# FitSNAP/FitSNAP

Measured on AMD Instinct MI355X. Metric: training rows/sec through A^T A + solve, 1000000 x 128 fp64 in total over the GPUs (strong scaling), higher is better.
Workload: dtype f64

## Files before the change

fitsnap_amd/build.py:

```python
from __future__ import annotations

import hashlib
import os
import shutil
import subprocess
import sys

HERE = os.path.dirname(os.path.abspath(__file__))
CSRC = os.path.join(HERE, "csrc")
LIBDIR = os.path.join(HERE, "_lib")
LIBNAME = "libfsnap_hip.so"
SOURCES = ["fsnap_syrk_quad.hip:0", "fsnap_syrk_quad.hip:1", "fsnap_syrk_quad.hip:2", "fsnap_syrk.hip", "fsnap_syrk_short.hip", "fsnap_rows.hip", "fsnap_chol.hip", "fsnap_trsm.hip", "fsnap_fused.hip", "fsnap_merr.hip", "fsnap_cand.hip", "fsnap_uq.hip", "fsnap_loco.hip", "fsnap_path.hip", "fsnap_joint.hip", "fsnap_select.hip", "fsnap_mcmc.hip", "fsnap_capi.cpp", "fsnap_comm.cpp", "fsnap_p2p.cpp",
           "fsnap_rowspace.cpp", "fsnap_rowspace_host.cpp", "fsnap_solve.cpp"]
HEADERS = ["fsnap_kernels.h", "fsnap_device_common.h", "fsnap_rowvar_body.h", "fsnap_ctx.h", "fsnap_rowspace_host.h", "fsnap_condest.h", "fsnap_p2p.h", os.path.join("..", "..", "include", "fsnap_hip.h")]
ARCH = "gfx950"


def lib_path() -> str:
    return os.path.join(LIBDIR, LIBNAME)


def _hipcc() -> str:
    exe = shutil.which("hipcc") or "/opt/rocm/bin/hipcc"
    if not os.path.exists(exe):
        raise RuntimeError("hipcc not found: libfsnap_hip.so cannot be built")
    return exe


def _source_digest() -> str:
    h = hashlib.sha256()
    for name in sorted({s.split(":")[0] for s in SOURCES}) + HEADERS:
        with open(os.path.join(CSRC, name), "rb") as f:
            h.update(f.read())
    return h.hexdigest()


def build_library(force: bool = False, verbose: bool = False) -> str:
    os.makedirs(LIBDIR, exist_ok=True)
    out = lib_path()
    stamp = out + ".sha256"
    digest = _source_digest()
    if not force and os.path.exists(out) and os.path.exists(stamp):
        with open(stamp) as f:
            if f.read().strip() == digest:
                return out
    hipcc = _hipcc()
    objs = []
    common = [f"--offload-arch={ARCH}", "-O3", "-std=c++17", "-fPIC", "-I", os.path.join(HERE, "..", "include")]
    procs = []
    objdir = os.path.join(LIBDIR, "obj")
    os.makedirs(objdir, exist_ok=True)
    hh = hashlib.sha256()
    for name in HEADERS:
        with open(os.path.join(CSRC, name), "rb") as f:
            hh.update(f.read())
    for entry in SOURCES:
        src, _, part = entry.partition(":")
        obj = os.path.join(objdir, os.path.splitext(src)[0] + (f"_{part}" if part else "") + ".o")
        cmd = [hipcc, *common]
        if part:
            cmd += [f"-DFSNAP_QUAD_PART={part}"]
        if src in ("fsnap_capi.cpp", "fsnap_comm.cpp", "fsnap_p2p.cpp", "fsnap_rowspace.cpp"):
            cmd += ["-x", "hip"]
        if src in ("fsnap_solve.cpp", "fsnap_rowspace_host.cpp"):
            cmd = [hipcc, "-x", "c++", "-O3", "-std=c++17", "-fPIC", "-mavx2", "-mfma",
                   "-I", os.path.join(HERE, "..", "include")]
        cmd += ["-c", os.path.join(CSRC, src), "-o", obj]
# ... 37 lines not shown
```

fitsnap_amd/csrc/fsnap_capi.cpp:

```cpp
#include <hip/hip_runtime.h>

#include <algorithm>
#include <cmath>
#include <atomic>
#include <chrono>
#include <cstdarg>
#include <cstdio>
#include <cstdlib>
#include <cstring>
#include <limits>
#include <new>
#include <queue>
#include <string>
#include <thread>
#include <vector>

#include "../../include/fsnap_hip.h"
#include "fsnap_kernels.h"

extern "C" int fsnap_solve_diag_tagged(int kind, double param, int64_t K, const double* G, const double* c, const double* diag,
                                       double* beta, int* rank, double* rcond_est, int upper, const void* owner,
                                       unsigned long long generation);
extern "C" int fsnap_solve_diag_upper(int kind, double param, int64_t K, const double* G, const double* c, const double* diag,
                                      double* beta, int* rank, double* rcond_est);
// ... 455 lines not shown
    return FSNAP_OK;
}

int launch_normal_eq_tiled(fsnap_ctx* ctx, double* d_packed, bool accumulate) {
    int rc;
    TiledGeometry g;
    if ((rc = plan_tiled(ctx, &g))) return rc;
    int npk = 0;
    if ((rc = ensure_wpack(ctx, &npk))) return rc;
    if (!ctx->part.ensure((size_t)g.nsplit * g.npairs * 4096 * sizeof(double)) ||
        !ctx->cpart.ensure((size_t)g.nsplit * g.NSB * 4 * 64 * sizeof(double)))
        return ctx->fail(FSNAP_E_NOMEM, "hipMalloc(partials) failed");
    fsnap::TiledArgs a;
    a.A = ctx->dA;
    a.lda = ctx->lda;
    a.wpack = ctx->wpack_override ? ctx->wpack_override : (const double*)ctx->wpack.p;
    a.m = ctx->m;
    a.K = (int)ctx->K;
    a.NSB = g.NSB;
    a.npairs = g.npairs;
    a.nsplit = g.nsplit;
    a.chunks_per_split = g.cps;
    a.nontemporal = false;
    a.part = (double*)ctx->part.p;
    a.cpart = (double*)ctx->cpart.p;
    a.spart = (const double*)ctx->wpack_spart.p;
    a.ns = npk;
    const int64_t cpart_key = ((int64_t)g.nsplit << 32) | (int64_t)g.NSB;
    if (ctx->cpart_key != cpart_key || ctx->cpart_ptr != ctx->cpart.p) {
        FSNAP_HIP(hipMemsetAsync(a.cpart, 0, (size_t)g.nsplit * g.NSB * 4 * 64 * sizeof(double), ctx->stream), "hipMemsetAsync");
        ctx->cpart_key = cpart_key;
        ctx->cpart_ptr = ctx->cpart.p;
    }
    hipEvent_t* evs;
    if ((rc = fit_events(ctx, &evs))) return rc;
    if (evs) FSNAP_HIP(hipEventRecord(evs[0], ctx->stream), "hipEventRecord");
    FSNAP_HIP(fsnap::launch_syrk_tiled(a, ctx->stream), "launch fsnap_syrk_tiled");
    if (evs) FSNAP_HIP(hipEventRecord(evs[1], ctx->stream), "hipEventRecord");
    FSNAP_HIP(fsnap::launch_reduce_tiled(a, d_packed, accumulate, ctx->stream), "launch fsnap_reduce_tiled");
    if (evs) FSNAP_HIP(hipEventRecord(evs[2], ctx->stream), "hipEventRecord");
    if (evs) ctx->t_syrk = true;
    return FSNAP_OK;
}

int launch_normal_eq(fsnap_ctx* ctx, double* d_packed, bool want_mirror = false, bool accumulate = false) {
    int rc;
    ctx->mirror_of = nullptr;
    ctx->chol_factor_of = nullptr;
    if ((rc = check_rows(ctx)) || (rc = check_weights(ctx))) return rc;
    if (use_tiled(ctx)) return launch_normal_eq_tiled(ctx, d_packed, accumulate);
    Geometry g;
    if ((rc = plan_geometry(ctx, &g))) return rc;
    const unsigned char* mask = ctx->dmask;
    if (!mask) {
        if ((rc = ensure_ones(ctx))) return rc;
        mask = (const unsigned char*)ctx->ones.p;
    }
    const int NT = g.NB * (g.NB + 1) / 2;
    const int cs_per_block = g.shortk ? 1 : 4 * g.cluster;
    if (!ctx->part.ensure((size_t)g.nblocks * NT * 256 * sizeof(double)) ||
        !ctx->cpart.ensure((size_t)g.nblocks * cs_per_block * g.NB * 16 * sizeof(double)) ||
        !ctx->spart.ensure((size_t)g.nblocks * cs_per_block * 4 * sizeof(double)))
        return ctx->fail(FSNAP_E_NOMEM, "hipMalloc(partials) failed");
    fsnap::SyrkArgs a;
    a.A = ctx->dA;
    a.lda = ctx->lda;
    a.b = ctx->db;
    a.w = ctx->dw;
    a.mask = mask;
    a.m = ctx->m;
    a.K = (int)ctx->K;
    a.nblocks = g.nblocks;
    a.split = g.split;
    a.chunks_per_wave = g.cpw;
    a.nontemporal = true;
    a.part = (double*)ctx->part.p;
    a.cpart = (double*)ctx->cpart.p;
    a.spart = (double*)ctx->spart.p;
    int ns = -1;
    const double* spart_src = a.spart;
    if (g.fused_pack) {
        a.fused_pack = true;
    } else {
        int npk = 0;
        if ((rc = ensure_wpack(ctx, &npk))) return rc;
        a.wpack = ctx->wpack_override ? ctx->wpack_override : (const double*)ctx->wpack.p;
        spart_src = (const double*)ctx->wpack_spart.p;
        ns = npk;
    }
    hipEvent_t* evs;
    if ((rc = fit_events(ctx, &evs))) return rc;
    if (evs) FSNAP_HIP(hipEventRecord(evs[0], ctx->stream), "hipEventRecord");
    if (g.quad && g.cluster > 1) {
        const size_t need = (size_t)g.nblocks * 4 * sizeof(int);
        if (ctx->quad_flow.bytes < need) {
            if (!ctx->quad_flow.ensure(need)) return ctx->fail(FSNAP_E_NOMEM, "hipMalloc(flow words) failed");
            FSNAP_HIP(hipMemsetAsync(ctx->quad_flow.p, 0, ctx->quad_flow.bytes, ctx->stream), "hipMemset(flow words)");
            ctx->quad_flow_tag = 0;
        }
        ctx->quad_flow_tag += 1u << 20;
        a.flow_words = (int*)ctx->quad_flow.p;
        const int flow = 2 | ((g.cluster == 2 ? 0 : 2) << 2);
        a.flow_tag = (int)(ctx->quad_flow_tag | (unsigned)flow);
    }
    if (g.shortk) FSNAP_HIP(fsnap::launch_syrk_short(a, ctx->stream), "launch fsnap_syrk_short");
    else if (g.quad) FSNAP_HIP(fsnap::launch_syrk_quad(a, ctx->stream), "launch fsnap_syrk_quad");
    else if (g.acc) FSNAP_HIP(fsnap::launch_syrk_acc(a, ctx->stream), "launch fsnap_syrk_acc");
// ... 2253 lines not shown
```

fitsnap_amd/csrc/fsnap_syrk.hip:

```cpp

#include <utility>

#include "fsnap_device_common.h"
#include "fsnap_kernels.h"

namespace {

__host__ __device__ constexpr int tri_index(int p, int q, int NB) {
    return p * NB - (p * (p - 1)) / 2 + (q - p);
}

__host__ __device__ inline int col_of(int bq, int e, int NB) {
    if ((NB & 1) && bq == NB - 1) return 16 * bq + e;
    return 32 * (bq >> 1) + 2 * e + (bq & 1);
}

__device__ __forceinline__ __amdgpu_buffer_rsrc_t make_rsrc(const void* p, unsigned bytes) {
    return __builtin_amdgcn_make_buffer_rsrc(const_cast<void*>(p), 0, (int)bytes, 0x00020000);
}

__device__ __forceinline__ double xlane_sum_rows(double x) {
    x += __shfl_xor(x, 16, 64);
    x += __shfl_xor(x, 32, 64);
    return x;
}

}

#ifdef FSNAP_TRACE
__device__ unsigned long long fsnap_trace_buf[4096 * 8];
__device__ unsigned long long fsnap_trace_wave[4096 * 16 * 4];
#define FSNAP_TRACE_CLK(v) const unsigned long long v = __builtin_readcyclecounter()
#endif

namespace {

template <int T, int NV>
__device__ __forceinline__ void acc_mfma(double a, double b, d4 (&vt)[NV]) {
    if constexpr (T < 32) {
        asm volatile("v_mfma_f64_16x16x4_f64 a[%2:%3], %0, %1, a[%2:%3]" : : "v"(a), "v"(b), "n"(8 * T), "n"(8 * T + 7));
    } else {
        asm volatile("v_mfma_f64_16x16x4_f64 %0, %1, %2, %0" : "+v"(vt[T - 32]) : "v"(a), "v"(b));
    }
}

template <int R>
__device__ __forceinline__ void acc_zero_reg() {
    asm volatile("v_accvgpr_write_b32 a[%0], 0" : : "n"(R));
}
template <int... R>
__device__ __forceinline__ void acc_zero_all(std::integer_sequence<int, R...>) {
    (acc_zero_reg<R>(), ...);
}

template <int T, int NV>
__device__ __forceinline__ d4 acc_read(const d4 (&vt)[NV]) {
    if constexpr (T >= 32) {
// ... 29 lines not shown

template <int NB>
struct RawM {
    u4 pr[NB / 2 > 0 ? NB / 2 : 1];
    u2 tail;
    u4 wp;
};

constexpr unsigned FSNAP_OOB_VOFF = 0xFFFFF000u;

struct WaveBufsP {
    __amdgpu_buffer_rsrc_t A, wp;
    unsigned voffA;
    unsigned voffT;
    unsigned voffP;
    unsigned chunk_bytes;
};

__device__ __forceinline__ u4 load_pack(const WaveBufsP& wb, unsigned cl) {
    return __builtin_amdgcn_raw_buffer_load_b128(wb.wp, wb.voffP, cl * 64u, 0);
}
__device__ __forceinline__ bool pack_keep(const u4& wp) {
    return ((wp[0] | (wp[1] & 0x7FFFFFFFu)) != 0u);
}

template <int NB, bool NT>
__device__ __forceinline__ void issue_rows(RawM<NB>& r, const WaveBufsP& wb, unsigned cl) {
    const unsigned soff = cl * wb.chunk_bytes;
    constexpr int AUX = NT ? 2 : 0;
    const bool keep = pack_keep(r.wp);
    const unsigned va = keep ? wb.voffA : FSNAP_OOB_VOFF;
#pragma unroll
    for (int j = 0; j < NB / 2; ++j) r.pr[j] = __builtin_amdgcn_raw_buffer_load_b128(wb.A, va + 256u * j, soff, AUX);
    if (NB & 1) {
        const unsigned vtl = keep ? wb.voffT : FSNAP_OOB_VOFF;
        r.tail = __builtin_amdgcn_raw_buffer_load_b64(wb.A, vtl, soff, AUX);
    }
}

template <int NB, bool NT>
__device__ __forceinline__ void issue_rows_w(RawM<NB>& r, const u4& wp, const WaveBufsP& wb, unsigned cl) {
    const unsigned soff = cl * wb.chunk_bytes;
    constexpr int AUX = NT ? 2 : 0;
    const bool keep = pack_keep(wp);
    const unsigned va = keep ? wb.voffA : FSNAP_OOB_VOFF;
#pragma unroll
    for (int j = 0; j < NB / 2; ++j) r.pr[j] = __builtin_amdgcn_raw_buffer_load_b128(wb.A, va + 256u * j, soff, AUX);
    if (NB & 1) {
        const unsigned vtl = keep ? wb.voffT : FSNAP_OOB_VOFF;
        r.tail = __builtin_amdgcn_raw_buffer_load_b64(wb.A, vtl, soff, AUX);
    }
}

template <class F, int... I>
__device__ __forceinline__ void wave_p_for_impl(F&& f, std::integer_sequence<int, I...>) {
    (f(std::integral_constant<int, I>{}), ...);
}
template <int N, class F>
__device__ __forceinline__ void wave_p_for(F&& f) {
    wave_p_for_impl(f, std::make_integer_sequence<int, N>{});
}

template <int NB, bool NT, int P>
__device__ __forceinline__ void issue_piece(RawM<NB>& r, const WaveBufsP& wb, unsigned cl, unsigned va, unsigned vtl) {
    constexpr int AUX = NT ? 2 : 0;
    constexpr int NPR = NB / 2;
    const unsigned soff = cl * wb.chunk_bytes;
    if (P < NPR) r.pr[P] = __builtin_amdgcn_raw_buffer_load_b128(wb.A, va + 256u * P, soff, AUX);
    if ((NB & 1) && P == NPR) r.tail = __builtin_amdgcn_raw_buffer_load_b64(wb.A, vtl, soff, AUX);
    static_assert(NPR + (NB & 1) <= NB, "one load piece per MFMA slot");
}

template <int NB, bool FULLK>
__device__ __forceinline__ double weighted_block(const RawM<NB>& r, int j, double wv, int K, int e) {
    if ((NB & 1) && j == NB - 1) {
        const double x = wv * __builtin_bit_cast(double, r.tail);
        if (FULLK) return x;
        return (16 * (NB - 1) + e < K) ? x : 0.0;
    }
    const double x = wv * __builtin_bit_cast(d2, r.pr[j >> 1])[j & 1];
    constexpr int last_pair = (NB & 1) ? -1 : NB / 2 - 1;
    if (FULLK || (j >> 1) != last_pair) return x;
    return (32 * (j >> 1) + 2 * e + (j & 1) < K) ? x : 0.0;
}

template <bool PACK>
__device__ __forceinline__ u4 load_pack_x(const WaveBufsP& wb, const double* lpk, unsigned cl) {
    if constexpr (PACK) return __builtin_bit_cast(u4, *reinterpret_cast<const d2*>(lpk + (size_t)cl * 8));
    else return load_pack(wb, cl);
}

__device__ __forceinline__ void pack_rows_to_lds(const double* __restrict__ b, const double* __restrict__ w,
                                                 const unsigned char* __restrict__ mask, int64_t row0, int64_t nrow,
                                                 unsigned wave_rows, unsigned region_rows, double* lpw, int lane, double* sout) {
    constexpr int PB = 16;
    const __amdgpu_buffer_rsrc_t rb = make_rsrc(b + row0, (unsigned)(nrow * 8));
    const __amdgpu_buffer_rsrc_t rw_ = make_rsrc(w + row0, (unsigned)(nrow * 8));
    const __amdgpu_buffer_rsrc_t rm = make_rsrc(mask + row0, (unsigned)nrow);
    double bb = 0.0, sb = 0.0, cnt = 0.0;
    for (unsigned r0 = 0; r0 < wave_rows; r0 += 64u * PB) {
        u2 bv[PB], wv[PB];
        unsigned char mk[PB];
#pragma unroll
        for (int u = 0; u < PB; ++u) {
            const unsigned row = r0 + 64u * u + (unsigned)lane;
            bv[u] = __builtin_amdgcn_raw_buffer_load_b64(rb, row * 8u, 0, 0);
            wv[u] = __builtin_amdgcn_raw_buffer_load_b64(rw_, row * 8u, 0, 0);
            mk[u] = __builtin_amdgcn_raw_buffer_load_b8(rm, row, 0, 0);
        }
#pragma unroll
        for (int u = 0; u < PB; ++u) {
            const unsigned row = r0 + 64u * u + (unsigned)lane;
            const bool keep = (mk[u] != 0);
            const double wvv = keep ? __builtin_bit_cast(double, wv[u]) : 0.0;
            const double wbv = keep ? wvv * __builtin_bit_cast(double, bv[u]) : 0.0;
            if (row < wave_rows) {
                d2 o;
                o[0] = wvv;
                o[1] = wbv;
                *reinterpret_cast<d2*>(lpw + (size_t)row * 2) = o;
            }
            bb = __builtin_fma(wbv, wbv, bb);
            sb += wbv;
            cnt += keep ? 1.0 : 0.0;
        }
    }
    for (unsigned row = wave_rows + (unsigned)lane; row < region_rows; row += 64u) {
        const d2 z = {0.0, 0.0};
        *reinterpret_cast<d2*>(lpw + (size_t)row * 2) = z;
    }
#pragma unroll
    for (int sh = 1; sh < 64; sh <<= 1) {
        bb += __shfl_xor(bb, sh, 64);
        sb += __shfl_xor(sb, sh, 64);
        cnt += __shfl_xor(cnt, sh, 64);
    }
    if (lane == 0) {
        sout[0] = bb;
        sout[1] = sb;
        sout[2] = cnt;
        sout[3] = 0.0;
    }
}

template <int NB, bool FULLK, bool NT, int P>
__device__ __forceinline__ void acc_slot(double (&V)[NB], const RawM<NB>& RN, double wv, double wbv, double& wbp, int K,
                                         int e, double (&cacc)[NB], RawM<NB>& RF, const WaveBufsP& wb, unsigned cl_fill,
                                         unsigned va, unsigned vtl) {
#if !defined(FSNAP_ACC_ABL) || !(FSNAP_ACC_ABL & 1)
    issue_piece<NB, NT, P>(RF, wb, cl_fill, va, vtl);
#endif
    if (P == 0) cacc[NB - 1] = __builtin_fma(V[NB - 1], wbp, cacc[NB - 1]);
    else cacc[P - 1] = __builtin_fma(V[P - 1], wbv, cacc[P - 1]);
    V[P] = weighted_block<NB, FULLK>(RN, P, wv, K, e);
    if (P == NB - 1) wbp = wbv;
    __builtin_amdgcn_sched_barrier(0);
}

template <int NB, bool FULLK, bool NT, bool PACK, int NV, int... P>
__device__ __forceinline__ void acc_step(double (&V)[NB], d4 (&vt)[NV], RawM<NB>& RF, const RawM<NB>& RN, const WaveBufsP& wb,
                                         const double* lpk, unsigned cl_fill, int K, int e, double (&cacc)[NB], double& wbp,
                                         const u4& PW, const u4& PKEEP, u4& PLOAD, std::integer_sequence<int, P...>) {
    const d2 wpn = __builtin_bit_cast(d2, PW);
    const double wv = wpn[0], wbv = wpn[1];
    const bool keep = pack_keep(PKEEP);
    const unsigned va = keep ? wb.voffA : FSNAP_OOB_VOFF;
    const unsigned vtl = (NB & 1) ? (keep ? wb.voffT : FSNAP_OOB_VOFF) : 0u;
#if !defined(FSNAP_ACC_ABL) || !(FSNAP_ACC_ABL & 1)
    PLOAD = load_pack_x<PACK>(wb, lpk, cl_fill + 2);
#endif
    __builtin_amdgcn_sched_barrier(0);
#if defined(FSNAP_ACC_ABL) && (FSNAP_ACC_ABL & 2)
    (acc_row<NB, P>(V, vt, std::make_integer_sequence<int, NB - P>{}), ...);
    (void)wbv;
#else
    ((acc_row<NB, P>(V, vt, std::make_integer_sequence<int, NB - P>{}),
      acc_slot<NB, FULLK, NT, P>(V, RN, wv, wbv, wbp, K, e, cacc, RF, wb, cl_fill, va, vtl)),
     ...);
#endif
}

constexpr int FSNAP_ACC_LDS_DOUBLES = 20480;
constexpr int FSNAP_ACC_PACK_PAD = 12;

}

template <int NB, bool FULLK, bool NT, bool PACK>
__global__ __launch_bounds__(256) __attribute__((amdgpu_waves_per_eu(1, 1))) void
fsnap_syrk_acc(const double* __restrict__ A, int64_t lda, const double* __restrict__ wpack, int64_t m, int K,
               int64_t chunks_per_wave, double* __restrict__ part, double* __restrict__ cpart,
               const double* __restrict__ bvec, const double* __restrict__ wvec, const unsigned char* __restrict__ mask,
               double* __restrict__ spart) {

    constexpr int NTILE = NB * (NB + 1) / 2;
    constexpr int NV = NTILE > 32 ? NTILE - 32 : 1;
    constexpr int NPART = (NTILE * 1024 + FSNAP_ACC_LDS_DOUBLES - 1) / FSNAP_ACC_LDS_DOUBLES;
    constexpr int PER = (NTILE + NPART - 1) / NPART;
    static_assert(4 * PER * 256 <= FSNAP_ACC_LDS_DOUBLES, "fold part does not fit the LDS");
    __shared__ __attribute__((aligned(16))) double lds[FSNAP_ACC_LDS_DOUBLES];
#ifdef FSNAP_TRACE
    const unsigned long long trace_t0 = wall_clock64();
    const unsigned long long trace_c0 = __builtin_readcyclecounter();
#endif
    const int lane = threadIdx.x & 63, e = lane & 15, kr = lane >> 4;
    const int rw = __builtin_amdgcn_readfirstlane((int)(threadIdx.x >> 6));
    const int64_t rowwave = (int64_t)blockIdx.x * 4 + rw;
    const int64_t nchunks = (m + 3) >> 2;
    int64_t c0 = rowwave * chunks_per_wave;
    int64_t c1 = c0 + chunks_per_wave;
    if (c1 > nchunks) c1 = nchunks;
    if (c0 > c1) c0 = c1;
    const int64_t row0 = c0 << 2;
    int64_t row1 = c1 << 2;
    if (row1 > m) row1 = m;
    const int64_t nrow = row1 > row0 ? row1 - row0 : 0;
    WaveBufsP wb;
    wb.A = make_rsrc(A + row0 * lda, (unsigned)(nrow * lda * 8 + (nrow ? 16 : 0)));
    wb.wp = make_rsrc(PACK ? nullptr : wpack + 2 * row0, PACK ? 0u : (unsigned)(nrow * 16));
    wb.voffA = (unsigned)((kr * lda + 2 * e) * 8);
    wb.voffT = (unsigned)((kr * lda + 16 * (NB - 1) + e) * 8);
    wb.voffP = (unsigned)(kr * 16);
    wb.chunk_bytes = (unsigned)(lda * 32);
    const unsigned ncl = (unsigned)(c1 - c0);

    const double* lpk = nullptr;
    if constexpr (PACK) {
        const unsigned wave_rows = (unsigned)chunks_per_wave * 4u;
        const unsigned region_rows = wave_rows + FSNAP_ACC_PACK_PAD * 4u;
        double* lpw = lds + (size_t)rw * region_rows * 2;
        pack_rows_to_lds(bvec, wvec, mask, row0, nrow, wave_rows, region_rows, lpw, lane, spart + rowwave * 4);
        lpk = lpw + 2 * kr;
    }

    asm volatile("" : : : "a0", "a255");
    acc_zero_all(std::make_integer_sequence<int, 256>{});
    d4 vt[NV];
#pragma unroll
    for (int u = 0; u < NV; ++u) vt[u] = d4{0.0, 0.0, 0.0, 0.0};
    double cacc[NB], V[NB];
#pragma unroll
    for (int p = 0; p < NB; ++p) cacc[p] = 0.0;
    RawM<NB> r0, r1, r2;
    constexpr auto rows = std::make_integer_sequence<int, NB>{};
    if (ncl > 0) {
        r0.wp = load_pack_x<PACK>(wb, lpk, 0);
        r1.wp = load_pack_x<PACK>(wb, lpk, 1);
        r2.wp = load_pack_x<PACK>(wb, lpk, 2);
        issue_rows<NB, NT>(r0, wb, 0);
        issue_rows<NB, NT>(r1, wb, 1);
        issue_rows<NB, NT>(r2, wb, 2);
        {
            const d2 wp0 = __builtin_bit_cast(d2, r0.wp);
            const double wv = wp0[0], wbv = wp0[1];
#pragma unroll
            for (int p = 0; p < NB; ++p) {
                V[p] = weighted_block<NB, FULLK>(r0, p, wv, K, e);
                cacc[p] = __builtin_fma(V[p], wbv, cacc[p]);
            }
        }
        u4 pk0 = r0.wp, pk1 = r1.wp, pk2 = r2.wp, pk3 = load_pack_x<PACK>(wb, lpk, 3), pk4 = load_pack_x<PACK>(wb, lpk, 4),
           pk5 = {0u, 0u, 0u, 0u};
        (void)pk0;
        double wbp = 0.0;
        unsigned cl = 0;
        for (; cl + 3 < ncl; cl += 6) {
            acc_step<NB, FULLK, NT, PACK>(V, vt, r0, r1, wb, lpk, cl + 3, K, e, cacc, wbp, pk1, pk3, pk5, rows);
            acc_step<NB, FULLK, NT, PACK>(V, vt, r1, r2, wb, lpk, cl + 4, K, e, cacc, wbp, pk2, pk4, pk0, rows);
            acc_step<NB, FULLK, NT, PACK>(V, vt, r2, r0, wb, lpk, cl + 5, K, e, cacc, wbp, pk3, pk5, pk1, rows);
            acc_step<NB, FULLK, NT, PACK>(V, vt, r0, r1, wb, lpk, cl + 6, K, e, cacc, wbp, pk4, pk0, pk2, rows);
            acc_step<NB, FULLK, NT, PACK>(V, vt, r1, r2, wb, lpk, cl + 7, K, e, cacc, wbp, pk5, pk1, pk3, rows);
            acc_step<NB, FULLK, NT, PACK>(V, vt, r2, r0, wb, lpk, cl + 8, K, e, cacc, wbp, pk0, pk2, pk4, rows);
        }
        if (cl < ncl) {
            acc_step<NB, FULLK, NT, PACK>(V, vt, r0, r1, wb, lpk, cl + 3, K, e, cacc, wbp, pk1, pk3, pk5, rows);
            acc_step<NB, FULLK, NT, PACK>(V, vt, r1, r2, wb, lpk, cl + 4, K, e, cacc, wbp, pk2, pk4, pk0, rows);
            acc_step<NB, FULLK, NT, PACK>(V, vt, r2, r0, wb, lpk, cl + 5, K, e, cacc, wbp, pk3, pk5, pk1, rows);
        }
        cacc[NB - 1] = __builtin_fma(V[NB - 1], wbp, cacc[NB - 1]);
    }
    asm volatile("s_nop 15\n\ts_nop 15\n\ts_nop 15" : "+v"(vt[0]));
#pragma unroll
    for (int u = 1; u < NV; ++u) asm volatile("" : "+v"(vt[u]));
#ifdef FSNAP_TRACE
    if (threadIdx.x == 0 && blockIdx.x < 4096) {
        const int64_t wg = blockIdx.x;
        fsnap_trace_buf[wg * 8 + 0] = trace_t0;
        fsnap_trace_buf[wg * 8 + 1] = wall_clock64();
        fsnap_trace_buf[wg * 8 + 2] = __builtin_amdgcn_s_getreg((31 << 11) | 4);
        fsnap_trace_buf[wg * 8 + 3] = __builtin_amdgcn_s_getreg((3 << 11) | 20);
        fsnap_trace_buf[wg * 8 + 4] = __builtin_readcyclecounter() - trace_c0;
    }
#endif

    if constexpr (PACK) __syncthreads();
    double* pw = part + (int64_t)blockIdx.x * (int64_t)(NTILE * 256);
    auto fold_part = [&](auto part_tag) {
        constexpr int H = decltype(part_tag)::value;
        constexpr int TB = H * PER;
        constexpr int NT_H = (TB + PER <= NTILE) ? PER : (NTILE - TB);
        constexpr int Q = (NT_H + 3) / 4;
        double* slot = lds + (size_t)rw * PER * 256;
        {
            d4 tmp[NT_H];
            acc_read_range<TB>(tmp, vt, std::make_integer_sequence<int, NT_H>{});
#pragma unroll
            for (int u = 0; u < NT_H; ++u)
#pragma unroll
                for (int i = 0; i < 4; ++i) slot[(u * 4 + i) * 64 + lane] = tmp[u][i];
        }
        __syncthreads();
        for (int u = rw * Q; u < (rw + 1) * Q && u < NT_H; ++u) {
#pragma unroll
            for (int i = 0; i < 4; ++i) {
                const int o = (u * 4 + i) * 64 + lane;
                const double s01 = lds[o] + lds[PER * 256 + o];
                pw[((TB + u) * 4 + i) * 64 + lane] = (s01 + lds[2 * PER * 256 + o]) + lds[3 * PER * 256 + o];
            }
        }
        if (H + 1 < NPART) __syncthreads();
    };
    wave_p_for<NPART>(fold_part);

    double* cw = cpart + rowwave * (int64_t)(NB * 16);
#pragma unroll
    for (int p = 0; p < NB; ++p) {
        double sm = xlane_sum_rows(cacc[p]);
        if (kr == 0) cw[p * 16 + e] = sm;
    }
#ifdef FSNAP_TRACE
    if (threadIdx.x == 0 && blockIdx.x < 4096) fsnap_trace_buf[blockIdx.x * 8 + 5] = wall_clock64();
#endif
}

constexpr int FSNAP_WAVE_P_PACK_PAD = 16;

template <int NB, bool FULLK, bool NT, bool PACK>
__global__ __launch_bounds__(256, 2) void fsnap_syrk_wave_p(const double* __restrict__ A, int64_t lda,
                                                            const double* __restrict__ wpack, int64_t m, int K,
                                                            int64_t chunks_per_wave,
                                                            double* __restrict__ part, double* __restrict__ cpart,
                                                            const double* __restrict__ bvec, const double* __restrict__ wvec,
                                                            const unsigned char* __restrict__ mask,
                                                            double* __restrict__ spart) {
    constexpr int NTILE = NB * (NB + 1) / 2;
    extern __shared__ __attribute__((aligned(16))) double lds[];
    const int lane = threadIdx.x & 63, e = lane & 15, kr = lane >> 4;
    const int rw = __builtin_amdgcn_readfirstlane((int)(threadIdx.x >> 6));
    const int64_t rowwave = (int64_t)blockIdx.x * 4 + rw;
    const int64_t nchunks = (m + 3) >> 2;
    int64_t c0 = rowwave * chunks_per_wave, ncl64;
    const int64_t stride = 1;
    {
        int64_t c1 = c0 + chunks_per_wave;
        if (c1 > nchunks) c1 = nchunks;
        if (c0 > c1) c0 = c1;
        ncl64 = c1 - c0;
    }
    const int64_t row0 = c0 << 2;
    int64_t row1 = (c0 + ncl64) << 2;
    if (row1 > m) row1 = m;
    const int64_t nrow = (ncl64 > 0 && row1 > row0) ? row1 - row0 : 0;
    WaveBufsP wb;
    wb.A = make_rsrc(A + row0 * lda, (unsigned)(nrow * lda * 8 + (nrow ? 16 : 0)));
    wb.wp = make_rsrc(PACK ? nullptr : wpack + 2 * row0, PACK ? 0u : (unsigned)(nrow * 16));
    wb.voffA = (unsigned)((kr * lda + 2 * e) * 8);
    wb.voffT = (unsigned)((kr * lda + 16 * (NB - 1) + e) * 8);
    wb.voffP = (unsigned)(kr * 16);
    wb.chunk_bytes = (unsigned)(stride * lda * 32);
    const unsigned pack_bytes = (unsigned)(stride * 64);
// ... 544 lines not shown
                const int split = q >> 2, wave = q & 3;
                s += src[((int64_t)split * NSB * 4 + wave) * 64];
            }
        } else {
            int p = g;
            double a0 = 0.0, a1 = 0.0, a2 = 0.0, a3 = 0.0;
            for (; p + 48 < np; p += 64) {
                const double x0 = src[(int64_t)p * stride], x1 = src[(int64_t)(p + 16) * stride];
                const double x2 = src[(int64_t)(p + 32) * stride], x3 = src[(int64_t)(p + 48) * stride];
                a0 += x0; a1 += x1; a2 += x2; a3 += x3;
            }
            for (; p < np; p += 16) a0 += src[(int64_t)p * stride];
            s = (a0 + a1) + (a2 + a3);
        }
    }
    red[tid] = s;
    __syncthreads();
    if (g == 0 && src) {
        double tot = 0.0;
#pragma unroll
        for (int k = 0; k < 16; ++k) tot += red[k * 64 + l];
        if (idx < nG) {
            reduce_tiled_store_g(idx, tot, NSB, K, out, accumulate);
        } else if (idx < nG + nC) {
            const int j = (int)(idx - nG);
            const int Ib = j >> 6, bq = (j >> 4) & 3, e = j & 15;
            const int cidx = 64 * Ib + 32 * (bq >> 1) + 2 * e + (bq & 1);
            if (cidx < K) out[(int64_t)K * K + cidx] = accumulate ? out[(int64_t)K * K + cidx] + tot : tot;
        } else {
            const int j = (int)(idx - nG - nC);
            if (j < 3) out[(int64_t)K * K + K + j] = accumulate ? out[(int64_t)K * K + K + j] + tot : tot;
        }
    }
}

namespace fsnap {

int syrk_num_blocks(int K) { return (K + 15) / 16; }

int syrk_waves_per_simd(int K, int split) {
    const int NB = syrk_num_blocks(K);
    const int ntw = (NB * (NB + 1) / 2 + split - 1) / split;
    const int regs = 8 * ntw + 12 * NB + 40;
    int wps = 512 / regs;
    if (wps < 1) wps = 1;
    if (wps > 8) wps = 8;
    return wps;
}

template <int NB>
static hipError_t launch_syrk_acc_nb(const SyrkArgs& a, hipStream_t st) {
    dim3 grid((unsigned)a.nblocks), block(256);
    const bool fullk = (a.K == 16 * NB);
    if (a.fused_pack ? (!a.b || !a.w || !a.mask || !a.spart) : !a.wpack) return hipErrorInvalidValue;
#define FSNAP_LAUNCH(FK, NTL, PK)                                                                                   \
    hipLaunchKernelGGL((fsnap_syrk_acc<NB, FK, NTL, PK>), grid, block, 0, st, a.A, a.lda, a.wpack, a.m, a.K,        \
                       a.chunks_per_wave, a.part, a.cpart, a.b, a.w, a.mask, a.spart)
#define FSNAP_LAUNCH_PK(FK, NTL)                 \
    do {                                         \
        if (a.fused_pack) FSNAP_LAUNCH(FK, NTL, true); \
        else FSNAP_LAUNCH(FK, NTL, false);       \
    } while (0)
    if (fullk) {
        if (a.nontemporal) FSNAP_LAUNCH_PK(true, true);
        else FSNAP_LAUNCH_PK(true, false);
    } else {
        if (a.nontemporal) FSNAP_LAUNCH_PK(false, true);
        else FSNAP_LAUNCH_PK(false, false);
    }
#undef FSNAP_LAUNCH_PK
#undef FSNAP_LAUNCH
    return hipGetLastError();
}

template <int NB>
static hipError_t launch_syrk_wave_p_nb(const SyrkArgs& a, hipStream_t st) {
    dim3 grid((unsigned)a.nblocks), block(256);
    const bool fullk = (a.K == 16 * NB);
    if (a.fused_pack ? (!a.b || !a.w || !a.mask || !a.spart) : !a.wpack) return hipErrorInvalidValue;
    constexpr size_t fold_bytes = (size_t)2 * (NB * (NB + 1) / 2) * 256 * sizeof(double);
    const size_t pair_bytes = a.fused_pack ? (size_t)4 * (size_t)(a.chunks_per_wave + FSNAP_WAVE_P_PACK_PAD) * 64 : 0;
    const size_t lds = pair_bytes > fold_bytes ? pair_bytes : fold_bytes;
    if (lds > 64 * 1024) return hipErrorInvalidValue;
#define FSNAP_LAUNCH(FK, NTL, PK)                                                                                      \
    hipLaunchKernelGGL((fsnap_syrk_wave_p<NB, FK, NTL, PK>), grid, block, lds, st, a.A, a.lda, a.wpack, a.m, a.K,       \
                       a.chunks_per_wave, a.part, a.cpart, a.b, a.w, a.mask, a.spart)
#define FSNAP_LAUNCH_PK(FK, NTL)                       \
    do {                                               \
        if (a.fused_pack) FSNAP_LAUNCH(FK, NTL, true); \
        else FSNAP_LAUNCH(FK, NTL, false);             \
    } while (0)
    if (fullk) {
        if (a.nontemporal) FSNAP_LAUNCH_PK(true, true);
        else FSNAP_LAUNCH_PK(true, false);
    } else {
        if (a.nontemporal) FSNAP_LAUNCH_PK(false, true);
        else FSNAP_LAUNCH_PK(false, false);
    }
#undef FSNAP_LAUNCH_PK
#undef FSNAP_LAUNCH
    return hipGetLastError();
}

int64_t syrk_wave_p_max_fused_cpw(int K, int wg_per_cu) {
    const int NB = syrk_num_blocks(K);
    const int64_t fold_bytes = (int64_t)2 * (NB * (NB + 1) / 2) * 256 * 8;
    int64_t budget = (int64_t)160 * 1024 / (wg_per_cu > 0 ? wg_per_cu : 1);
    if (budget > 64 * 1024) budget = 64 * 1024;
    if (budget < fold_bytes) budget = fold_bytes;
    return budget / 256 - FSNAP_WAVE_P_PACK_PAD;
}

hipError_t launch_syrk_wave_p(const SyrkArgs& a, hipStream_t st) {
    switch (syrk_num_blocks(a.K)) {
        case 1: return launch_syrk_wave_p_nb<1>(a, st);
        case 2: return launch_syrk_wave_p_nb<2>(a, st);
        case 3: return launch_syrk_wave_p_nb<3>(a, st);
        case 4: return launch_syrk_wave_p_nb<4>(a, st);
        case 5: return launch_syrk_wave_p_nb<5>(a, st);
        default: return hipErrorInvalidValue;
    }
}

int64_t syrk_acc_max_fused_cpw() { return FSNAP_ACC_LDS_DOUBLES / 32 - FSNAP_ACC_PACK_PAD; }

hipError_t launch_syrk_acc(const SyrkArgs& a, hipStream_t st) {
    switch (syrk_num_blocks(a.K)) {
        case 6: return launch_syrk_acc_nb<6>(a, st);
        case 7: return launch_syrk_acc_nb<7>(a, st);
        case 8: return launch_syrk_acc_nb<8>(a, st);
        case 9: return launch_syrk_acc_nb<9>(a, st);
        default: return hipErrorInvalidValue;
// ... 44 lines not shown
```

Measured before the change: 3.124 billion.

## Overlap row prefetch with pack, drop mask gating when all rows kept

In the fused-pack accumulation kernel, the first three chunks of A rows are now prefetched before the b/w pack stage, and accumulator zeroing is interleaved with the pack loads so their latency overlaps. When no mask is supplied, the pack no longer reads a ones-mask buffer. If every weight in the wave is nonzero, the main loop runs a variant without per-step keep gating, up to a precomputed safe bound. The LDS partial fold is also vectorised to two-double loads. This adds template instantiations, register pressure and subtle bound logic for the ungated region.

```diff
diff --git a/fitsnap_amd/build.py b/fitsnap_amd/build.py
--- a/fitsnap_amd/build.py
+++ b/fitsnap_amd/build.py
@@ -12,7 +12,7 @@
 LIBNAME = "libfsnap_hip.so"
 SOURCES = ["fsnap_syrk_quad.hip:0", "fsnap_syrk_quad.hip:1", "fsnap_syrk_quad.hip:2", "fsnap_syrk.hip", "fsnap_syrk_short.hip", "fsnap_rows.hip", "fsnap_chol.hip", "fsnap_trsm.hip", "fsnap_fused.hip", "fsnap_merr.hip", "fsnap_cand.hip", "fsnap_uq.hip", "fsnap_loco.hip", "fsnap_path.hip", "fsnap_joint.hip", "fsnap_select.hip", "fsnap_mcmc.hip", "fsnap_capi.cpp", "fsnap_comm.cpp", "fsnap_p2p.cpp",
            "fsnap_rowspace.cpp", "fsnap_rowspace_host.cpp", "fsnap_solve.cpp"]
-HEADERS = ["fsnap_kernels.h", "fsnap_device_common.h", "fsnap_rowvar_body.h", "fsnap_ctx.h", "fsnap_rowspace_host.h", "fsnap_condest.h", "fsnap_p2p.h", os.path.join("..", "..", "include", "fsnap_hip.h")]
+HEADERS = ["fsnap_kernels.h", "fsnap_syrk_plan.h", "fsnap_device_common.h", "fsnap_rowvar_body.h", "fsnap_ctx.h", "fsnap_rowspace_host.h", "fsnap_condest.h", "fsnap_p2p.h", os.path.join("..", "..", "include", "fsnap_hip.h")]
 ARCH = "gfx950"
 
 
diff --git a/fitsnap_amd/csrc/fsnap_capi.cpp b/fitsnap_amd/csrc/fsnap_capi.cpp
--- a/fitsnap_amd/csrc/fsnap_capi.cpp
+++ b/fitsnap_amd/csrc/fsnap_capi.cpp
@@ -531,7 +531,8 @@
     Geometry g;
     if ((rc = plan_geometry(ctx, &g))) return rc;
     const unsigned char* mask = ctx->dmask;
-    if (!mask) {
+    const bool mask_optional = g.fused_pack && (g.acc || g.packed);
+    if (!mask && !mask_optional) {
         if ((rc = ensure_ones(ctx))) return rc;
         mask = (const unsigned char*)ctx->ones.p;
     }
diff --git a/fitsnap_amd/csrc/fsnap_syrk.hip b/fitsnap_amd/csrc/fsnap_syrk.hip
--- a/fitsnap_amd/csrc/fsnap_syrk.hip
+++ b/fitsnap_amd/csrc/fsnap_syrk.hip
@@ -1,8 +1,10 @@
 
+#include <type_traits>
 #include <utility>
 
 #include "fsnap_device_common.h"
 #include "fsnap_kernels.h"
+#include "fsnap_syrk_plan.h"
 
 namespace {
 
@@ -138,6 +140,27 @@
     }
 }
 
+template <int NB, bool NT>
+__device__ __forceinline__ void issue_rows_raw(RawM<NB>& r, const WaveBufsP& wb, unsigned cl) {
+    const unsigned soff = cl * wb.chunk_bytes;
+    constexpr int AUX = NT ? 2 : 0;
+#pragma unroll
+    for (int j = 0; j < NB / 2; ++j) r.pr[j] = __builtin_amdgcn_raw_buffer_load_b128(wb.A, wb.voffA + 256u * j, soff, AUX);
+    if (NB & 1) r.tail = __builtin_amdgcn_raw_buffer_load_b64(wb.A, wb.voffT, soff, AUX);
+}
+template <int NB>
+__device__ __forceinline__ void sanitize_rows(RawM<NB>& r) {
+    const bool keep = pack_keep(r.wp);
+#pragma unroll
+    for (int j = 0; j < NB / 2; ++j)
+#pragma unroll
+        for (int i = 0; i < 4; ++i) r.pr[j][i] = keep ? r.pr[j][i] : 0u;
+    if (NB & 1) {
+        r.tail[0] = keep ? r.tail[0] : 0u;
+        r.tail[1] = keep ? r.tail[1] : 0u;
+    }
+}
+
 template <class F, int... I>
 __device__ __forceinline__ void wave_p_for_impl(F&& f, std::integer_sequence<int, I...>) {
     (f(std::integral_constant<int, I>{}), ...);
@@ -176,28 +199,37 @@
     else return load_pack(wb, cl);
 }
 
-__device__ __forceinline__ void pack_rows_to_lds(const double* __restrict__ b, const double* __restrict__ w,
-                                                 const unsigned char* __restrict__ mask, int64_t row0, int64_t nrow,
-                                                 unsigned wave_rows, unsigned region_rows, double* lpw, int lane, double* sout) {
-    constexpr int PB = 16;
-    const __amdgpu_buffer_rsrc_t rb = make_rsrc(b + row0, (unsigned)(nrow * 8));
-    const __amdgpu_buffer_rsrc_t rw_ = make_rsrc(w + row0, (unsigned)(nrow * 8));
-    const __amdgpu_buffer_rsrc_t rm = make_rsrc(mask + row0, (unsigned)nrow);
+template <bool MASK>
+struct PackRows {
+    static constexpr int PB = 16;
+    __amdgpu_buffer_rsrc_t rb, rw_, rm;
+    unsigned nrow, wave_rows;
+    u2 bv[PB], wv[PB];
+    unsigned char mk[PB];
     double bb = 0.0, sb = 0.0, cnt = 0.0;
-    for (unsigned r0 = 0; r0 < wave_rows; r0 += 64u * PB) {
-        u2 bv[PB], wv[PB];
-        unsigned char mk[PB];
+    bool zero_w = false;
+
+    __device__ __forceinline__ PackRows(const double* __restrict__ b, const double* __restrict__ w,
+                                        const unsigned char* __restrict__ mask, int64_t row0, int64_t nrow_, unsigned wave_rows_)
+        : rb(make_rsrc(b + row0, (unsigned)(nrow_ * 8))), rw_(make_rsrc(w + row0, (unsigned)(nrow_ * 8))),
+          rm(make_rsrc(MASK ? mask + row0 : nullptr, MASK ? (unsigned)nrow_ : 0u)), nrow((unsigned)nrow_),
+          wave_rows(wave_rows_) {}
+
+    __device__ __forceinline__ void issue(unsigned r0, int lane) {
 #pragma unroll
         for (int u = 0; u < PB; ++u) {
             const unsigned row = r0 + 64u * u + (unsigned)lane;
             bv[u] = __builtin_amdgcn_raw_buffer_load_b64(rb, row * 8u, 0, 0);
             wv[u] = __builtin_amdgcn_raw_buffer_load_b64(rw_, row * 8u, 0, 0);
-            mk[u] = __builtin_amdgcn_raw_buffer_load_b8(rm, row, 0, 0);
-        }
+            if constexpr (MASK) mk[u] = __builtin_amdgcn_raw_buffer_load_b8(rm, row, 0, 0);
+        }
+    }
+
+    __device__ __forceinline__ void finish(unsigned r0, double* lpw, int lane) {
 #pragma unroll
         for (int u = 0; u < PB; ++u) {
             const unsigned row = r0 + 64u * u + (unsigned)lane;
-            const bool keep = (mk[u] != 0);
+            const bool keep = MASK ? (mk[u] != 0) : (row < nrow);
             const double wvv = keep ? __builtin_bit_cast(double, wv[u]) : 0.0;
             const double wbv = keep ? wvv * __builtin_bit_cast(double, bv[u]) : 0.0;
             if (row < wave_rows) {
@@ -206,27 +238,50 @@
                 o[1] = wbv;
                 *reinterpret_cast<d2*>(lpw + (size_t)row * 2) = o;
             }
+            const u2 wbits = __builtin_bit_cast(u2, wvv);
+            zero_w |= (row < nrow) && ((wbits[0] | (wbits[1] & 0x7FFFFFFFu)) == 0u);
             bb = __builtin_fma(wbv, wbv, bb);
             sb += wbv;
             cnt += keep ? 1.0 : 0.0;
         }
     }
-    for (unsigned row = wave_rows + (unsigned)lane; row < region_rows; row += 64u) {
-        const d2 z = {0.0, 0.0};
-        *reinterpret_cast<d2*>(lpw + (size_t)row * 2) = z;
-    }
-#pragma unroll
-    for (int sh = 1; sh < 64; sh <<= 1) {
-        bb += __shfl_xor(bb, sh, 64);
-        sb += __shfl_xor(sb, sh, 64);
-        cnt += __shfl_xor(cnt, sh, 64);
-    }
-    if (lane == 0) {
-        sout[0] = bb;
-        sout[1] = sb;
-        sout[2] = cnt;
-        sout[3] = 0.0;
-    }
+
+    __device__ __forceinline__ void close(unsigned region_rows, double* lpw, int lane, double* sout) {
+        for (unsigned row = wave_rows + (unsigned)lane; row < region_rows; row += 64u) {
+            const d2 z = {0.0, 0.0};
+            *reinterpret_cast<d2*>(lpw + (size_t)row * 2) = z;
+        }
+#pragma unroll
+        for (int sh = 1; sh < 64; sh <<= 1) {
+            bb += __shfl_xor(bb, sh, 64);
+            sb += __shfl_xor(sb, sh, 64);
+            cnt += __shfl_xor(cnt, sh, 64);
+        }
+        if (lane == 0) {
+            sout[0] = bb;
+            sout[1] = sb;
+            sout[2] = cnt;
+            sout[3] = 0.0;
+        }
+    }
+
+    __device__ __forceinline__ bool all_keep() const { return __builtin_amdgcn_ballot_w64(zero_w) == 0ull; }
+};
+
+__device__ __forceinline__ void pack_rows_to_lds(const double* __restrict__ b, const double* __restrict__ w,
+                                                 const unsigned char* __restrict__ mask, int64_t row0, int64_t nrow,
+                                                 unsigned wave_rows, unsigned region_rows, double* lpw, int lane, double* sout) {
+    auto run = [&](auto has_mask) __attribute__((always_inline)) {
+        using Pack = PackRows<decltype(has_mask)::value>;
+        Pack pk(b, w, mask, row0, nrow, wave_rows);
+        for (unsigned r0 = 0; r0 < wave_rows; r0 += 64u * Pack::PB) {
+            pk.issue(r0, lane);
+            pk.finish(r0, lpw, lane);
+        }
+        pk.close(region_rows, lpw, lane, sout);
+    };
+    if (mask) run(std::true_type{});
+    else run(std::false_type{});
 }
 
 template <int NB, bool FULLK, bool NT, int P>
@@ -243,13 +298,13 @@
     __builtin_amdgcn_sched_barrier(0);
 }
 
-template <int NB, bool FULLK, bool NT, bool PACK, int NV, int... P>
+template <int NB, bool FULLK, bool NT, bool PACK, bool GATE, int NV, int... P>
 __device__ __forceinline__ void acc_step(double (&V)[NB], d4 (&vt)[NV], RawM<NB>& RF, const RawM<NB>& RN, const WaveBufsP& wb,
                                          const double* lpk, unsigned cl_fill, int K, int e, double (&cacc)[NB], double& wbp,
                                          const u4& PW, const u4& PKEEP, u4& PLOAD, std::integer_sequence<int, P...>) {
     const d2 wpn = __builtin_bit_cast(d2, PW);
     const double wv = wpn[0], wbv = wpn[1];
-    const bool keep = pack_keep(PKEEP);
+    const bool keep = GATE ? pack_keep(PKEEP) : true;
     const unsigned va = keep ? wb.voffA : FSNAP_OOB_VOFF;
     const unsigned vtl = (NB & 1) ? (keep ? wb.voffT : FSNAP_OOB_VOFF) : 0u;
 #if !defined(FSNAP_ACC_ABL) || !(FSNAP_ACC_ABL & 1)
@@ -309,32 +364,57 @@
     wb.chunk_bytes = (unsigned)(lda * 32);
     const unsigned ncl = (unsigned)(c1 - c0);
 
+    const fsnap::AccEndsPlan plan = fsnap::acc_ends_plan(nrow, ncl, lda, NB);
+    const unsigned early = PACK ? plan.early : 0u;
+
+    RawM<NB> r0, r1, r2;
     const double* lpk = nullptr;
+    bool all_keep = false;
     if constexpr (PACK) {
+        if (early > 0) issue_rows_raw<NB, NT>(r0, wb, 0);
+        if (early > 1) issue_rows_raw<NB, NT>(r1, wb, 1);
+        if (early > 2) issue_rows_raw<NB, NT>(r2, wb, 2);
+        __builtin_amdgcn_sched_barrier(0);
         const unsigned wave_rows = (unsigned)chunks_per_wave * 4u;
         const unsigned region_rows = wave_rows + FSNAP_ACC_PACK_PAD * 4u;
         double* lpw = lds + (size_t)rw * region_rows * 2;
-        pack_rows_to_lds(bvec, wvec, mask, row0, nrow, wave_rows, region_rows, lpw, lane, spart + rowwave * 4);
+        auto pack = [&](auto has_mask) __attribute__((always_inline)) {
+            using Pack = PackRows<decltype(has_mask)::value>;
+            Pack pk(bvec, wvec, mask, row0, nrow, wave_rows);
+            pk.issue(0u, lane);
+            __builtin_amdgcn_sched_barrier(0);
+            asm volatile("" : : : "a0", "a255");
+            acc_zero_all(std::make_integer_sequence<int, 256>{});
+            __builtin_amdgcn_sched_barrier(0);
+            pk.finish(0u, lpw, lane);
+            for (unsigned rb0 = 64u * Pack::PB; rb0 < wave_rows; rb0 += 64u * Pack::PB) {
+                pk.issue(rb0, lane);
+                pk.finish(rb0, lpw, lane);
+            }
+            pk.close(region_rows, lpw, lane, spart + rowwave * 4);
+            all_keep = pk.all_keep();
+        };
+        if (mask) pack(std::true_type{});
+        else pack(std::false_type{});
         lpk = lpw + 2 * kr;
-    }
-
-    asm volatile("" : : : "a0", "a255");
-    acc_zero_all(std::make_integer_sequence<int, 256>{});
+    } else {
+        asm volatile("" : : : "a0", "a255");
+        acc_zero_all(std::make_integer_sequence<int, 256>{});
+    }
     d4 vt[NV];
 #pragma unroll
     for (int u = 0; u < NV; ++u) vt[u] = d4{0.0, 0.0, 0.0, 0.0};
     double cacc[NB], V[NB];
 #pragma unroll
     for (int p = 0; p < NB; ++p) cacc[p] = 0.0;
-    RawM<NB> r0, r1, r2;
     constexpr auto rows = std::make_integer_sequence<int, NB>{};
     if (ncl > 0) {
         r0.wp = load_pack_x<PACK>(wb, lpk, 0);
         r1.wp = load_pack_x<PACK>(wb, lpk, 1);
         r2.wp = load_pack_x<PACK>(wb, lpk, 2);
-        issue_rows<NB, NT>(r0, wb, 0);
-        issue_rows<NB, NT>(r1, wb, 1);
-        issue_rows<NB, NT>(r2, wb, 2);
+        if (early > 0) { if (!all_keep) sanitize_rows<NB>(r0); } else issue_rows<NB, NT>(r0, wb, 0);
+        if (early > 1) { if (!all_keep) sanitize_rows<NB>(r1); } else issue_rows<NB, NT>(r1, wb, 1);
+        if (early > 2) { if (!all_keep) sanitize_rows<NB>(r2); } else issue_rows<NB, NT>(r2, wb, 2);
         {
             const d2 wp0 = __builtin_bit_cast(d2, r0.wp);
             const double wv = wp0[0], wbv = wp0[1];
@@ -348,20 +428,24 @@
            pk5 = {0u, 0u, 0u, 0u};
         (void)pk0;
         double wbp = 0.0;
+#define FSNAP_ACC_TRIP3(G)                                                                                               \
+    acc_step<NB, FULLK, NT, PACK, G>(V, vt, r0, r1, wb, lpk, cl + 3, K, e, cacc, wbp, pk1, pk3, pk5, rows);            \
+    acc_step<NB, FULLK, NT, PACK, G>(V, vt, r1, r2, wb, lpk, cl + 4, K, e, cacc, wbp, pk2, pk4, pk0, rows);            \
+    acc_step<NB, FULLK, NT, PACK, G>(V, vt, r2, r0, wb, lpk, cl + 5, K, e, cacc, wbp, pk3, pk5, pk1, rows)
+#define FSNAP_ACC_TRIP6(G)                                                                                               \
+    FSNAP_ACC_TRIP3(G);                                                                                                  \
+    acc_step<NB, FULLK, NT, PACK, G>(V, vt, r0, r1, wb, lpk, cl + 6, K, e, cacc, wbp, pk4, pk0, pk2, rows);            \
+    acc_step<NB, FULLK, NT, PACK, G>(V, vt, r1, r2, wb, lpk, cl + 7, K, e, cacc, wbp, pk5, pk1, pk3, rows);            \
+    acc_step<NB, FULLK, NT, PACK, G>(V, vt, r2, r0, wb, lpk, cl + 8, K, e, cacc, wbp, pk0, pk2, pk4, rows)
         unsigned cl = 0;
-        for (; cl + 3 < ncl; cl += 6) {
-            acc_step<NB, FULLK, NT, PACK>(V, vt, r0, r1, wb, lpk, cl + 3, K, e, cacc, wbp, pk1, pk3, pk5, rows);
-            acc_step<NB, FULLK, NT, PACK>(V, vt, r1, r2, wb, lpk, cl + 4, K, e, cacc, wbp, pk2, pk4, pk0, rows);
-            acc_step<NB, FULLK, NT, PACK>(V, vt, r2, r0, wb, lpk, cl + 5, K, e, cacc, wbp, pk3, pk5, pk1, rows);
-            acc_step<NB, FULLK, NT, PACK>(V, vt, r0, r1, wb, lpk, cl + 6, K, e, cacc, wbp, pk4, pk0, pk2, rows);
-            acc_step<NB, FULLK, NT, PACK>(V, vt, r1, r2, wb, lpk, cl + 7, K, e, cacc, wbp, pk5, pk1, pk3, rows);
-            acc_step<NB, FULLK, NT, PACK>(V, vt, r2, r0, wb, lpk, cl + 8, K, e, cacc, wbp, pk0, pk2, pk4, rows);
-        }
-        if (cl < ncl) {
-            acc_step<NB, FULLK, NT, PACK>(V, vt, r0, r1, wb, lpk, cl + 3, K, e, cacc, wbp, pk1, pk3, pk5, rows);
-            acc_step<NB, FULLK, NT, PACK>(V, vt, r1, r2, wb, lpk, cl + 4, K, e, cacc, wbp, pk2, pk4, pk0, rows);
-            acc_step<NB, FULLK, NT, PACK>(V, vt, r2, r0, wb, lpk, cl + 5, K, e, cacc, wbp, pk3, pk5, pk1, rows);
-        }
+        if constexpr (PACK) {
+            const unsigned ung_end = all_keep ? plan.ung_end : 0u;
+            for (; cl < ung_end; cl += 6) { FSNAP_ACC_TRIP6(false); }
+        }
+        for (; cl < plan.full_end; cl += 6) { FSNAP_ACC_TRIP6(true); }
+        if (plan.half) { FSNAP_ACC_TRIP3(true); }
+#undef FSNAP_ACC_TRIP6
+#undef FSNAP_ACC_TRIP3
         cacc[NB - 1] = __builtin_fma(V[NB - 1], wbp, cacc[NB - 1]);
     }
     asm volatile("s_nop 15\n\ts_nop 15\n\ts_nop 15" : "+v"(vt[0]));
@@ -397,10 +481,15 @@
         __syncthreads();
         for (int u = rw * Q; u < (rw + 1) * Q && u < NT_H; ++u) {
 #pragma unroll
-            for (int i = 0; i < 4; ++i) {
-                const int o = (u * 4 + i) * 64 + lane;
-                const double s01 = lds[o] + lds[PER * 256 + o];
-                pw[((TB + u) * 4 + i) * 64 + lane] = (s01 + lds[2 * PER * 256 + o]) + lds[3 * PER * 256 + o];
+            for (int h = 0; h < 2; ++h) {
+                const int o = u * 256 + h * 128 + 2 * lane;
+                const d2 s0 = *reinterpret_cast<const d2*>(lds + o), s1 = *reinterpret_cast<const d2*>(lds + PER * 256 + o);
+                const d2 s2 = *reinterpret_cast<const d2*>(lds + 2 * PER * 256 + o);
+                const d2 s3 = *reinterpret_cast<const d2*>(lds + 3 * PER * 256 + o);
+                d2 t;
+                t[0] = ((s0[0] + s1[0]) + s2[0]) + s3[0];
+                t[1] = ((s0[1] + s1[1]) + s2[1]) + s3[1];
+                *reinterpret_cast<d2*>(pw + (TB * 256 + o)) = t;
             }
         }
         if (H + 1 < NPART) __syncthreads();
@@ -1051,7 +1140,7 @@
 static hipError_t launch_syrk_acc_nb(const SyrkArgs& a, hipStream_t st) {
     dim3 grid((unsigned)a.nblocks), block(256);
     const bool fullk = (a.K == 16 * NB);
-    if (a.fused_pack ? (!a.b || !a.w || !a.mask || !a.spart) : !a.wpack) return hipErrorInvalidValue;
+    if (a.fused_pack ? (!a.b || !a.w || !a.spart) : !a.wpack) return hipErrorInvalidValue;
 #define FSNAP_LAUNCH(FK, NTL, PK)                                                                                   \
     hipLaunchKernelGGL((fsnap_syrk_acc<NB, FK, NTL, PK>), grid, block, 0, st, a.A, a.lda, a.wpack, a.m, a.K,        \
                        a.chunks_per_wave, a.part, a.cpart, a.b, a.w, a.mask, a.spart)
@@ -1076,7 +1165,7 @@
 static hipError_t launch_syrk_wave_p_nb(const SyrkArgs& a, hipStream_t st) {
     dim3 grid((unsigned)a.nblocks), block(256);
     const bool fullk = (a.K == 16 * NB);
-    if (a.fused_pack ? (!a.b || !a.w || !a.mask || !a.spart) : !a.wpack) return hipErrorInvalidValue;
+    if (a.fused_pack ? (!a.b || !a.w || !a.spart) : !a.wpack) return hipErrorInvalidValue;
     constexpr size_t fold_bytes = (size_t)2 * (NB * (NB + 1) / 2) * 256 * sizeof(double);
     const size_t pair_bytes = a.fused_pack ? (size_t)4 * (size_t)(a.chunks_per_wave + FSNAP_WAVE_P_PACK_PAD) * 64 : 0;
     const size_t lds = pair_bytes > fold_bytes ? pair_bytes : fold_bytes;
diff --git a/fitsnap_amd/csrc/fsnap_syrk_plan.h b/fitsnap_amd/csrc/fsnap_syrk_plan.h
--- /dev/null
+++ b/fitsnap_amd/csrc/fsnap_syrk_plan.h
@@ -0,0 +1,35 @@
+#pragma once
+
+#include <cstdint>
+
+#if defined(__HIPCC__)
+#define FSNAP_PLAN_HD __host__ __device__
+#else
+#define FSNAP_PLAN_HD
+#endif
+
+namespace fsnap {
+
+struct AccEndsPlan {
+    unsigned safe;
+    unsigned early;
+    unsigned ung_end;
+    unsigned full_end;
+    bool half;
+};
+
+FSNAP_PLAN_HD constexpr unsigned acc_plan_steps(const AccEndsPlan& p) { return p.full_end + (p.half ? 3u : 0u); }
+
+FSNAP_PLAN_HD constexpr AccEndsPlan acc_ends_plan(int64_t nrow, unsigned ncl, int64_t lda, int NB) {
+    AccEndsPlan p{0u, 0u, 0u, 0u, false};
+    const int64_t over = lda > 0 ? (16 * (int64_t)NB + lda - 1) / lda : 0;
+    const int64_t safe = (lda > 0 && over >= 1 && nrow + 1 >= over + 4) ? (nrow + 1 - over) / 4 : 0;
+    p.safe = (unsigned)(safe < (int64_t)ncl ? safe : (int64_t)ncl);
+    p.early = p.safe < 3u ? p.safe : 3u;
+    p.ung_end = p.safe >= 9u ? 6u * ((p.safe - 3u) / 6u) : 0u;
+    p.full_end = ncl > 3u ? 6u * ((ncl - 3u + 5u) / 6u) : 0u;
+    p.half = p.full_end < ncl;
+    return p;
+}
+
+}
```

Result: no change. 3.152 billion, median of 3 (+0.9%).
